# anibali/dsnt-pose2d

Measured on AMD Instinct MI355X. Metric: images/sec (train step, 256x256, 16 joints), higher is better.
Workload: dtype f32; 1 GPU; hg2 + DSNT + JS reg, 256x256 -> 64x64x16, batch 32 per GPU, RMSprop lr 2.5e-4, train step fwd+loss+bwd+optim; global_batch=32, parallelism=dp1, launches_fwd=212

## Files before the change

dsnt-pose2d_amd/csrc/elementwise.hip:

```cpp
#include "common.h"
#include <string.h>
#include "bn_pro.h"
#include "conv_split.h"
#include "ew_bodies.h"
#include "stage.h"

static inline int tile_cgs(long tiles, int C4) { return tiles < 256 && C4 > 16 && C4 % 16 == 0 ? 16 : (C4 < 256 ? C4 : 256); }
static inline unsigned tile_grid_y(long tiles, int C4) { const int c = tile_cgs(tiles, C4); return c == 16 && C4 > 16 ? C4 / 16 : 1; }

template <int MODE>
__global__ __launch_bounds__(256) void tile_reduce_kernel(
    const float* __restrict__ a, const float* __restrict__ x, const float* __restrict__ scale,
    const float* __restrict__ shift, const float* __restrict__ mean,
    const float* __restrict__ invstd, int relu, float* __restrict__ partial, long M, int C, int cgs,
    const float* __restrict__ ymask = nullptr, float* __restrict__ dz_out = nullptr) {
    __shared__ float red[256 * 8];
    const int tid = threadIdx.x;
    const int C4 = C >> 2;
    const int rpar = 256 / cgs;
    const int cg_l = tid % cgs, rl = tid / cgs;
    const bool active = rl < rpar;
    const long row0 = (long)blockIdx.x * TILE_ROWS;
    const long row1 = row0 + TILE_ROWS < M ? row0 + TILE_ROWS : M;
    for (int cg0 = blockIdx.y * cgs; cg0 < C4; cg0 += cgs * gridDim.y) {
// ... 294 lines not shown
        DSNT_LAUNCH_OP(DSNT_ST_APPLY, bn_act_bwd_apply_kernel<false>, dim3(grid), dim3(256), 0, stream, ap);
    DSNT_CHECK_LAUNCH("dsnt_bn_act_bwd_apply");
}

extern "C" int dsnt_bn_act_bwd_apply_pro(const float* da, const float* x, const float* scale, const float* shift,
                                         const float* mean, const float* invstd, const float* partial, int ntiles,
                                         float* dgamma, float* dbeta, int accumulate_params, float* coef, int relu,
                                         float* dx, int accumulate, int64_t M, int C, float* amax, void* stream) {
    DSNT_REQUIRE(partial && ntiles > 0 && coef && C <= 256 && (long)ntiles * C <= 16384, DSNT_ERR_ARG,
                 "dsnt_bn_act_bwd_apply_pro: needs partial sums of at most 256 channels / 128 KB and a coef buffer");
    BnBwdProP q;
    q.partial = partial; q.tiles = ntiles; q.C = C; q.invM = 1.0 / (double)M;
    q.dgamma = dgamma; q.dbeta = dbeta; q.accumulate = accumulate_params; q.coef = coef;
    return bn_act_bwd_apply_impl(da, x, scale, shift, mean, invstd, coef, relu, dx, accumulate, M, C, amax, stream, &q);
}
extern "C" int dsnt_bn_act_bwd_apply_base(const float* da, const float* x, const float* scale, const float* shift,
                                          const float* mean, const float* invstd, const float* coef, int relu,
                                          const float* base, float* dx, int64_t M, int C, float* amax, void* stream) {
    DSNT_REQUIRE(base && base != dx, DSNT_ERR_ARG, "dsnt_bn_act_bwd_apply_base: `base` must be a second tensor");
    return bn_act_bwd_apply_impl(da, x, scale, shift, mean, invstd, coef, relu, dx, 1, M, C, amax, stream, nullptr, base);
}
extern "C" int dsnt_bn_act_bwd_apply_pro_base(const float* da, const float* x, const float* scale, const float* shift,
                                              const float* mean, const float* invstd, const float* partial, int ntiles,
                                              float* dgamma, float* dbeta, int accumulate_params, float* coef, int relu,
                                              const float* base, float* dx, int64_t M, int C, float* amax, void* stream) {
    DSNT_REQUIRE(base && base != dx, DSNT_ERR_ARG, "dsnt_bn_act_bwd_apply_pro_base: `base` must be a second tensor");
    DSNT_REQUIRE(partial && ntiles > 0 && coef && C <= 256 && (long)ntiles * C <= 16384, DSNT_ERR_ARG,
                 "dsnt_bn_act_bwd_apply_pro_base: needs partial sums of at most 256 channels / 128 KB and a coef buffer");
    BnBwdProP q;
    q.partial = partial; q.tiles = ntiles; q.C = C; q.invM = 1.0 / (double)M;
    q.dgamma = dgamma; q.dbeta = dbeta; q.accumulate = accumulate_params; q.coef = coef;
    return bn_act_bwd_apply_impl(da, x, scale, shift, mean, invstd, coef, relu, dx, 1, M, C, amax, stream, &q, base);
}
__global__ void maxpool2_fwd_kernel(const float4* __restrict__ x, float4* __restrict__ y,
                                    uchar4* __restrict__ idx, int N, int H, int W, int C4) {
    const int Ho = H >> 1, Wo = W >> 1;
    const long total = (long)N * Ho * Wo * C4;
    for (long i = (long)blockIdx.x * blockDim.x + threadIdx.x; i < total;
         i += (long)gridDim.x * blockDim.x) {
        const int cg = (int)(i % C4);
        long t = i / C4;
        const int ow = (int)(t % Wo); t /= Wo;
        const int oh = (int)(t % Ho);
        const int n = (int)(t / Ho);
        const float4* base = x + (((long)n * H + 2 * oh) * W + 2 * ow) * C4 + cg;
        const float4 v0 = base[0], v1 = base[C4], v2 = base[(long)W * C4], v3 = base[(long)W * C4 + C4];
        float4 m = v0;
        uchar4 k = make_uchar4(0, 0, 0, 0);
#define POOL_STEP(V, P)                                  \
        if (V.x > m.x || V.x != V.x) { m.x = V.x; k.x = P; } \
        if (V.y > m.y || V.y != V.y) { m.y = V.y; k.y = P; } \
        if (V.z > m.z || V.z != V.z) { m.z = V.z; k.z = P; } \
        if (V.w > m.w || V.w != V.w) { m.w = V.w; k.w = P; }
        POOL_STEP(v1, 1) POOL_STEP(v2, 2) POOL_STEP(v3, 3)
#undef POOL_STEP
        y[i] = m;
        idx[i] = k;
    }
}

extern "C" int dsnt_maxpool2_fwd(const float* x, float* y, uint8_t* idx, int N, int H, int W, int C,
                                 void* stream) {
    DSNT_REQUIRE(x && y && idx && N > 0 && H > 0 && W > 0 && C > 0, DSNT_ERR_ARG, "dsnt_maxpool2_fwd: bad argument");
    DSNT_REQUIRE(H % 2 == 0 && W % 2 == 0, DSNT_ERR_SHAPE, "dsnt_maxpool2_fwd: H and W must be even (got %dx%d)", H, W);
    DSNT_REQUIRE(C % 4 == 0 && dsnt_aligned16(x) && dsnt_aligned16(y) && (((uintptr_t)idx) & 3) == 0,
                 DSNT_ERR_ALIGN, "dsnt_maxpool2_fwd: alignment");
// ... 548 lines not shown
```

dsnt-pose2d_amd/csrc/ew_bodies.h:

```cpp
#pragma once
#include "common.h"
#include "bn_pro.h"

#define TILE_ROWS 128

struct TileOpP {
    const float* a; const float* b; float* y; unsigned char* idx; float* partial;
    int N, Ho, Wo, C, cgs;
    OutBoundsP tail;
    const float* bn_scale; const float* bn_shift; int bn_relu;
};
template <int OP>
__device__ __forceinline__ void tile_op_stats_body(const TileOpP& q, const int bx, const int by, const int gy, float* red) {
    const float* __restrict__ a = q.a; const float* __restrict__ b = q.b; float* __restrict__ y = q.y;
    unsigned char* __restrict__ idx = q.idx; float* partial = q.partial;
    const int N = q.N, Ho = q.Ho, Wo = q.Wo, C = q.C, cgs = q.cgs;
    const OutBoundsP tail = q.tail;
    const float* __restrict__ bn_scale = q.bn_scale; const float* __restrict__ bn_shift = q.bn_shift; const int bn_relu = q.bn_relu;
    const int tid = threadIdx.x;
    const int C4 = C >> 2;
    const int rpar = 256 / cgs;
    const int cg_l = tid % cgs, rl = tid / cgs;
    const bool active = rl < rpar;
    const long M = (long)N * Ho * Wo;
// ... 93 lines not shown
                for (int e = 0; e < 8; ++e) acc[e] += red[(j * cgs + tid) * 8 + e];
            float* p0 = partial + ((size_t)bx * 2 + 0) * C + (size_t)(cg0 + tid) * 4;
            float* p1 = partial + ((size_t)bx * 2 + 1) * C + (size_t)(cg0 + tid) * 4;
            *reinterpret_cast<float4*>(p0) = make_float4(acc[0], acc[1], acc[2], acc[3]);
            *reinterpret_cast<float4*>(p1) = make_float4(acc[4], acc[5], acc[6], acc[7]);
        }
    }
    if (tail.amax) amax_commit(am, tail.amax, 0, bx);
    if (tail.amax_bn) amax_commit(am2, tail.amax_bn, 1, bx);
}

template <int OP>
__global__ __launch_bounds__(256) void tile_op_stats_kernel(TileOpP q) {
    __shared__ __attribute__((aligned(16))) float red[256 * 8];
    tile_op_stats_body<OP>(q, blockIdx.x, blockIdx.y, gridDim.y, red);
}

struct BnApplyVec { float4 sc, sh, mu, is, c0, c1; };
__device__ __forceinline__ float4 bn_apply_one(const float4 g, const float4 xv, const BnApplyVec& v, int relu) {
    float4 dz = g;
    if (relu) {
        if (fmaf(xv.x, v.sc.x, v.sh.x) <= 0.f) dz.x = 0.f;
        if (fmaf(xv.y, v.sc.y, v.sh.y) <= 0.f) dz.y = 0.f;
        if (fmaf(xv.z, v.sc.z, v.sh.z) <= 0.f) dz.z = 0.f;
        if (fmaf(xv.w, v.sc.w, v.sh.w) <= 0.f) dz.w = 0.f;
    }
    float4 o;
    o.x = v.sc.x * (dz.x - v.c0.x - (xv.x - v.mu.x) * v.is.x * v.c1.x);
    o.y = v.sc.y * (dz.y - v.c0.y - (xv.y - v.mu.y) * v.is.y * v.c1.y);
    o.z = v.sc.z * (dz.z - v.c0.z - (xv.z - v.mu.z) * v.is.z * v.c1.z);
    o.w = v.sc.w * (dz.w - v.c0.w - (xv.w - v.mu.w) * v.is.w * v.c1.w);
    return o;
}
struct BnApplyP {
    const float4* da; const float4* x; const float4* scale; const float4* shift; const float4* mean; const float4* invstd;
    const float4* coef; int relu; float4* dx; const float4* base; long n4; int C4; unsigned* amax; BnBwdProP pro;
};
template <bool FIXED>
__device__ __forceinline__ void bn_act_bwd_apply_body(const BnApplyP& q, const int vb, const int vgrid, double* pro_sh, const bool finalise) {
    const float4* __restrict__ da = q.da; const float4* __restrict__ x = q.x; const float4* __restrict__ scale = q.scale;
    const float4* __restrict__ shift = q.shift; const float4* __restrict__ mean = q.mean; const float4* __restrict__ invstd = q.invstd;
    const float4* coef = q.coef; const int relu = q.relu; float4* dx = q.dx; const float4* base = q.base;
    const long n4 = q.n4; const int C4 = q.C4; unsigned* __restrict__ amax = q.amax; const BnBwdProP pro = q.pro;
    const bool accumulate = base != nullptr;
    if (pro.partial && finalise) {
        bn_pro_backward<256>(pro, pro_sh, vb == 0);
        __syncthreads();
    }
    float am = 0.f;
    const long stride = (long)vgrid * 256;
    long i = threadIdx.x < 256 ? (long)vb * 256 + threadIdx.x : n4;
    auto vec = [&](int cg) {
        BnApplyVec v;
        v.sc = scale[cg]; v.sh = shift[cg]; v.mu = mean[cg]; v.is = invstd[cg]; v.c0 = coef[cg]; v.c1 = coef[C4 + cg];
        return v;
    };
    auto amx = [&](const float4 o) { am = fmaxf(fmaxf(fmaxf(fabsf(o.x), fabsf(o.y)), fmaxf(fabsf(o.z), fabsf(o.w))), am); };
    if (FIXED) {
        const BnApplyVec v = vec((int)((i < n4 ? i : 0) % C4));
        for (; i + stride < n4; i += 2 * stride) {
            const float4 g0 = da[i], x0 = x[i], g1 = da[i + stride], x1 = x[i + stride];
            float4 p0 = make_float4(0.f, 0.f, 0.f, 0.f), p1 = p0;
            if (accumulate) { p0 = base[i]; p1 = base[i + stride]; }
            float4 o0 = bn_apply_one(g0, x0, v, relu), o1 = bn_apply_one(g1, x1, v, relu);
            if (accumulate) {
                o0.x += p0.x; o0.y += p0.y; o0.z += p0.z; o0.w += p0.w;
                o1.x += p1.x; o1.y += p1.y; o1.z += p1.z; o1.w += p1.w;
            }
            dx[i] = o0; dx[i + stride] = o1;
            amx(o0); amx(o1);
        }
        if (i < n4) {
            float4 o = bn_apply_one(da[i], x[i], v, relu);
            if (accumulate) { const float4 p = base[i]; o.x += p.x; o.y += p.y; o.z += p.z; o.w += p.w; }
            dx[i] = o;
            amx(o);
        }
    } else {
        for (; i < n4; i += stride) {
            float4 o = bn_apply_one(da[i], x[i], vec((int)(i % C4)), relu);
            if (accumulate) { const float4 p = base[i]; o.x += p.x; o.y += p.y; o.z += p.z; o.w += p.w; }
            dx[i] = o;
            amx(o);
        }
    }
    if (amax) amax_commit(am, amax, 0, vb);
}

template <bool FIXED>
__global__ void bn_act_bwd_apply_kernel(BnApplyP q) {
    __shared__ double pro_sh[512];
    bn_act_bwd_apply_body<FIXED>(q, blockIdx.x, gridDim.x, pro_sh, true);
}

struct PoolBwdP { const float4* dy; const uchar4* idx; float4* dx; int accumulate; const float4* extra; int N, H, W, C4; unsigned* amax; };
__device__ __forceinline__ void maxpool2_bwd_body(const PoolBwdP& q, const int vb, const int vgrid) {
    const float4* __restrict__ dy = q.dy; const uchar4* __restrict__ idx = q.idx; float4* dx = q.dx; const int accumulate = q.accumulate;
    const float4* __restrict__ extra = q.extra; const int H = q.H, W = q.W, C4 = q.C4, N = q.N; unsigned* amax = q.amax;
    const int Ho = H >> 1, Wo = W >> 1;
    const long total = (long)N * Ho * Wo * C4;
    float am = 0.f;
    for (long i = threadIdx.x < 256 ? (long)vb * 256 + threadIdx.x : total; i < total; i += (long)vgrid * 256) {
        const int cg = (int)(i % C4);
        long t = i / C4;
        const int ow = (int)(t % Wo); t /= Wo;
        const int oh = (int)(t % Ho);
        const int n = (int)(t / Ho);
        const float4 g = dy[i];
        const uchar4 k = idx[i];
        float4* base = dx + (((long)n * H + 2 * oh) * W + 2 * ow) * C4 + cg;
#pragma unroll
        for (int p = 0; p < 4; ++p) {
            float4* q = base + (p >> 1) * (long)W * C4 + (p & 1) * C4;
            float4 o = make_float4(k.x == p ? g.x : 0.f, k.y == p ? g.y : 0.f, k.z == p ? g.z : 0.f,
                                   k.w == p ? g.w : 0.f);
            if (accumulate) { const float4 c = *q; o.x += c.x; o.y += c.y; o.z += c.z; o.w += c.w; }
            if (extra) { const float4 e = extra[q - dx]; o.x += e.x; o.y += e.y; o.z += e.z; o.w += e.w; }
            *q = o;
            am = fmaxf(fmaxf(fmaxf(fabsf(o.x), fabsf(o.y)), fmaxf(fabsf(o.z), fabsf(o.w))), am);
        }
    }
    if (amax) amax_commit(am, amax, 0, vb);
}

struct UpBwdP { const float4* dout; float4* dlow; int accumulate; int N, H, W, C4; unsigned* amax; };
// ... 124 lines not shown
```

dsnt-pose2d_amd/dsnt/_lib.py:

```python
import ctypes as C
import os

import torch

_HERE = os.path.dirname(os.path.abspath(__file__))
LIB_PATH = os.environ.get('DSNT_HIP_LIB') or os.path.join(os.path.dirname(_HERE), 'csrc', 'libdsnt_hip.so')

P = C.c_void_p
I = C.c_int
L = C.c_int64
F = C.c_float
D = C.c_double


class ConvGeom(C.Structure):
    _fields_ = [(n, C.c_int) for n in
                ('N', 'H', 'W', 'Cin', 'Ho', 'Wo', 'Cout', 'R', 'S', 'stride', 'pad', 'dil')]


GP = C.POINTER(ConvGeom)


class BnBwdEpilogue(C.Structure):
    _fields_ = [('x', C.c_void_p), ('scale', C.c_void_p), ('shift', C.c_void_p), ('mean', C.c_void_p),
# ... 63 lines not shown
    'dsnt_conv_fwd_bf16x6_ex': [P, P, L, P, P, P, P, I, P, P, P, GP, BP, TP, P],
    'dsnt_conv_pack_dgrad': [P, P, I, I, I, I, P],
    'dsnt_conv_pack_dgrad_all': [P, I, P, P, P, L, P],
    'dsnt_conv_fwd_bf16x6': [P, P, L, P, P, P, P, I, P, P, P, GP, P],
    'dsnt_split_bf16x3': [P, P, L, P],
    'dsnt_conv_fwd_f16x3_ex': [P, P, L, P, P, P, P, P, P, I, P, P, P, GP, BP, TP, P],
    'dsnt_conv_fwd_f16x3_stream': [P, P, L, P, P, P, P, P, P, I, P, P, P, GP, BP, TP, P],
    'dsnt_amax': [P, L, P, P],
    'dsnt_split_f16x2': [P, P, L, L, P, P],
    'dsnt_f16_prep_weights': [P, I, I, P],
    'dsnt_f16_prep_bn_bounds': [P, I, P],
    'dsnt_conv_wgrad': [P, P, P, I, P, P, P, P, I, GP, P],
    'dsnt_conv_wgrad_bf16x6': [P, P, P, I, P, P, P, P, I, GP, P],
    'dsnt_conv_wgrad_f16x3': [P, P, P, I, P, P, P, P, I, P, P, GP, P],
    'dsnt_conv1x1_fwd_f16x3': [P, P, L, P, P, P, P, P, P, I, P, P, GP, TP, P],
    'dsnt_conv1x1_bwd_f16x3': [BP, P, AP, P, L, P, P, P, P, P, P, P, I, GP, P],
    'dsnt_conv_dgrad_f16x3_stream_apply': [P, AP, P, P, L, P, P, P, P, I, GP, BP, TP, P],
    'dsnt_wgrad_reduce_all': [P, I, I, P],
    'dsnt_conv_wgrad_group': [P, I, I, P],
    'dsnt_bn_stats': [P, P, L, I, P],
    'dsnt_bn_finalize': [P, I, L, I, P, P, P, P, F, F, I, P, P, P, P, P],
    'dsnt_bn_act_fwd': [P, P, P, I, P, L, I, P],
    'dsnt_bn_act_bwd_reduce': [P, P, P, P, P, P, I, P, L, I, P],
    'dsnt_bn_bwd_finalize': [P, I, L, I, P, P, I, P, P],
    'dsnt_bn_bwd_finalize_bound': [P, I, L, I, P, P, I, P, P, P, P, P],
    'dsnt_bn_eval_prep': [P, I, P],
    'dsnt_bn_act_bwd_apply': [P, P, P, P, P, P, P, I, P, I, L, I, P],
    'dsnt_bn_act_bwd_apply_amax': [P, P, P, P, P, P, P, I, P, I, L, I, P, P],
    'dsnt_bn_act_bwd_apply_pro': [P, P, P, P, P, P, P, I, P, P, I, P, I, P, I, L, I, P, P],
    'dsnt_stem4_fwd_f16x3': [P, P, L, P, P, P, P, P, GP, TP, P],
    'dsnt_bn_add_act_bwd_reduce': [P, P, P, P, P, I, P, P, L, I, P],
    'dsnt_bn_act_bwd_apply_base': [P, P, P, P, P, P, P, I, P, P, L, I, P, P],
    'dsnt_bn_act_bwd_apply_pro_base': [P, P, P, P, P, P, P, I, P, P, I, P, I, P, P, L, I, P, P],
    'dsnt_conv_fwd_pro': [P, P, P, P, PP, I, P, P, P, GP, TP, P],
    'dsnt_fill_zero': [P, L, P],
    'dsnt_axpy_amax': [P, P, F, I, L, P, P],
    'dsnt_maxpool2_bwd_amax': [P, P, P, I, I, I, I, I, P, P],
    'dsnt_maxpool2_bwd_add': [P, P, P, I, P, I, I, I, I, P, P],
    'dsnt_upsample2_bwd_amax': [P, P, I, I, I, I, I, P, P],
    'dsnt_maxpool2_fwd': [P, P, P, I, I, I, I, P],
    'dsnt_maxpool2_bwd': [P, P, P, I, I, I, I, I, P],
    'dsnt_maxpool2_fwd_stats': [P, P, P, P, I, I, I, I, TP, P],
    'dsnt_upsample2_add_fwd_stats': [P, P, P, P, I, I, I, I, TP, P],
    'dsnt_bn_act_fwd_stats': [P, P, P, I, P, P, L, I, TP, P],
    'dsnt_s2d_input': [P, P, I, I, I, I, TP, P],
    'dsnt_s2d_weights': [P, P, I, I, P],
    'dsnt_s2d_weights_prep': [P, P, P, P, P, I, P],
    'dsnt_maxpool3s2_fwd': [P, P, P, I, I, I, I, P],
    'dsnt_maxpool3s2_bwd': [P, P, P, I, I, I, I, I, P],
    'dsnt_bn_add_act_fwd': [P, P, P, P, I, P, L, I, P],
    'dsnt_relu_bwd': [P, P, P, L, P],
    'dsnt_zero_insert': [P, P, I, I, I, I, I, I, I, P],
    'dsnt_conv_dgrad_strided': [P, P, P, P, P, GP, BP, TP, P],
    'dsnt_upsample2_add_fwd': [P, P, P, I, I, I, I, P],
    'dsnt_upsample2_bwd': [P, P, I, I, I, I, I, P],
    'dsnt_axpy': [P, P, F, I, L, P],
    'dsnt_nchw_to_nhwc': [P, P, I, I, I, I, P],
    'dsnt_nhwc_to_nchw': [P, P, I, I, I, I, P],
    'dsnt_rmsprop_step': [P, P, P, L, F, F, F, F, F, P],
    'dsnt_sgd_step': [P, P, P, L, F, F, F, F, I, P],
    'dsnt_rmsprop_step_guarded': [P, P, P, L, F, F, F, F, F, P, P],
    'dsnt_sgd_step_guarded': [P, P, P, L, F, F, F, F, I, P, P],
    'dsnt_nonfinite_flag': [P, L, P, I, P],
    'dsnt_pckh': [P, P, P, P, P, P, F, P, P, I, I, P],
    'dsnt_pckh_hist': [P, P, P, P, P, P, P, I, P, P, I, I, P],
    'dsnt_augment_fwd': [P, I, I, I, P, P, P, P, I, C.c_uint64, C.c_uint64, P, P, P, P],
# ... 115 lines not shown
```

dsnt-pose2d_amd/dsnt/engine.py:

```python
import ctypes as C
import os

import torch

from . import _lib
from ._lib import ConvGeom, BnBwdEpilogue, BnTail, BnPrologue, BnBwdApply

BN_EPS = 1e-5
BN_MOMENTUM = 0.1


class Act:
    __slots__ = ('buf', 'N', 'H', 'W', 'C', '_grad', 'stats', 'name', 'grad_amax', 'amax_tail', 'fold_ok',
                 'pending_apply', 'uses', 'gives_away', 'is_branch', 'grad_shared', 'pending_add', 'base', 'base_amax')

    def __init__(self, buf, name=''):
        self.buf = buf
        self.N, self.H, self.W, self.C = buf.shape
        self._grad = None
        self.base, self.base_amax = None, None
        self.stats = None
        self.amax_tail = None
        self.grad_amax = None
        self.fold_ok = False
        self.pending_apply = None
        self.uses = 0
        self.gives_away = False
        self.is_branch = False
        self.grad_shared = False
        self.pending_add = None
        self.name = name

    @property
    def M(self):
        return self.N * self.H * self.W

    @property
    def grad(self):
        if self._grad is None and self.base is not None:
            self._grad, self.grad_amax, self.grad_shared = self.base, self.base_amax, True
        return self._grad

    @grad.setter
    def grad(self, g):
        self._grad = g


class ConvParams:
    __slots__ = ('w', 'b', 'gw', 'gb', 'Cout', 'R', 'S', 'Cin', 'stride', 'pad', 'dil', 'wq', 'wq_stride', 'wq16', 'wb',
                 'post_reduce')

    def __init__(self, w, b, gw, gb, stride=1, pad=0, dil=1):
        self.w, self.b, self.gw, self.gb = w, b, gw, gb
        self.wq, self.wq_stride = None, 0
        self.wq16, self.wb = None, None
        self.post_reduce = None
        self.Cout, self.R, self.S, self.Cin = w.shape
        self.stride, self.pad, self.dil = stride, pad, dil


class BnParams:
    __slots__ = ('gamma', 'beta', 'ggamma', 'gbeta', 'rmean', 'rvar', 'C', 'uses', 'momentum', 'eps')

# ... 13 lines not shown
    def __init__(self, device, training, record=None):
        self.device = device
        self.training = training
        self.record = training if record is None else bool(record)
        self.fwd = []
        self.bwd = []
        self._bwd_emitters = []
        self._scratch = {}
        self._keep = []
        self.lib = _lib.load()
        self.nbytes = 0
        self.bytes_fwd, self.bytes_bwd, self.bytes_by_name, self._ws_ptrs = 0, 0, {}, set()
        self.use_bf16x6 = os.environ.get('DSNT_MFMA', 'bf16x6') != 'f32'
        self.bf16x6_min_rows = int(os.environ.get('DSNT_BF16X6_MIN_ROWS', '4096'))
        self.lane = 0
        self.use_lanes = os.environ.get('DSNT_LANES', '1') != '0'
        self.fuse_join = True
        self.side_stream = None
        self.wgrad_stream = None
        self.side_lanes = (1, 3)
        self.n_lanes = 3 + len(self.side_lanes) - 1
        self.chain_lanes = (0,) + self.side_lanes
        self.more_streams = ()
        self.wgrad_lane = 2 if (self.use_lanes and os.environ.get('DSNT_WGRAD_LANE', '1') != '0') else None
        self.wgrad_lane_rows = int(os.environ.get('DSNT_X_WGRAD_LANE_ROWS', '16000'))
        self.wgrad_lane_res = False
        self.wgrad_lane_from = self.chain_lanes
        self.conv3s = 'conv3s' not in os.environ.get('DSNT_OFF', '').replace('+', ',').split(',')
        self.bwd1 = 'bwd1' not in os.environ.get('DSNT_OFF', '').replace('+', ',').split(',')
        self.fwd1 = 'fwd1' not in os.environ.get('DSNT_OFF', '').replace('+', ',').split(',')
        self.fold3 = 'fold3' not in os.environ.get('DSNT_OFF', '').replace('+', ',').split(',')
        self.fold3_rows = int(os.environ.get('DSNT_X_FOLD3_ROWS', '16384'))
        self.stem4 = 'stem4' not in os.environ.get('DSNT_OFF', '').replace('+', ',').split(',')
        self.stage = os.environ.get('DSNT_STAGE', '0') == '1'
        self.stage_min_run = int(os.environ.get('DSNT_X_STAGE_MIN_RUN', '3'))
        self.stage_max_vgrid = int(os.environ.get('DSNT_X_STAGE_MAX_VGRID', '512'))
        self.stage_grid = int(os.environ.get('DSNT_X_STAGE_GRID', '64'))
        self.stage_census = []
        self._f16_w_stream = {}
        self.conv_share = True
        self.wgrad_share = True
        self._x = dict(kv.split('=') for kv in os.environ.get('DSNT_X', '').split(',') if '=' in kv)
        self.wgrad_narrow = self._x.get('wgrad_narrow', '1')
        self.share_grads = self._x.get('share_grads', '1') != '0'
        self.defer_res = self._x.get('defer_res', '1') != '0'
        self.flush_points = self._x.get('flush_points', '1') != '0'
        self.prep_split = self._x.get('prep_split', '1') != '0'
        self.cur_bucket = 0
        self._wgrad_lane_reads = set()
        self._writer_base = None
        self._ident = None
        self.release_rows = int(os.environ.get('DSNT_X_RELEASE_ROWS', '4096'))
        self._release_total, self._release_left = 0, 0
        self._held = []
        self.acts = []
        self.dgrad_slots = []
        self.dgrad_total = 0
        self.dgrad_f32 = None
        self.dgrad_planes = None
        self.param_arena = None
        self.defer_reduce = os.environ.get('DSNT_DEFER_REDUCE', '1') != '0'
        self._pending_reduce = []
        self.group_rows = int(os.environ.get('DSNT_X_GROUP_ROWS', '8192')) if self.defer_reduce else 0
        self._pending_group = []
        self.fuse_op_stats = True
        self.fuse_finalize = os.environ.get('DSNT_FUSE_FINALIZE', '1') != '0'
        self.fuse_finalize_max = int(os.environ.get('DSNT_X_FUSE_FINALIZE_MAX', '2048'))
        self.use_f16x3 = self.use_bf16x6 and os.environ.get('DSNT_SPLIT', 'f16x3') == 'f16x3'
        if self.record and not self.training:
            self.use_f16x3 = False
        self._f16_w_rows, self._f16_w_seen = [], set()
        self._f16_bn_rows = []
        self._eval_bn_rows = []
        self._amax_buf, self._amax_used = None, 0
        self.raw_f16 = True
        self._planar_src, self._prep_exempt, self._post_reduce = {}, set(), []
        self.stem_s2d_on = True
        self._famax_buf, self._famax_used, self._famax_of, self._famax_bn_of = None, 0, {}, {}
        self.amax_all = True
        self._f16_dw_rows = []
        self._dgrad_pack = None
        self.prep_on_side_lane = self.use_lanes
        self.dgrad_planes16, self.dgrad_bounds = None, None
        self.f16_uses = []
        self._pending_group_uses = []
        self.c_replay = True
        self._clists = {}

    def empty(self, *shape, dtype=torch.float32):
        t = torch.empty(*shape, device=self.device, dtype=dtype)
        self.nbytes += t.numel() * t.element_size()
        self._keep.append(t)
        return t

    def scratch(self, key, numel):
        if False:
            return self.empty(max(numel, 1))
        key = (key, self.lane)
        t = self._scratch.get(key)
        if t is None or t.numel() < numel:
            if t is not None:
                self._keep.append(t)
            t = torch.empty(max(numel, 1), device=self.device, dtype=torch.float32)
            self.nbytes += t.numel() * 4
            self._scratch[key] = t
        return t

    def scratch_bf16(self, key, numel):
        key = (key, self.lane)
        t = self._scratch.get(key)
        if t is None or t.numel() < numel:
            if t is not None:
                self._keep.append(t)
            t = torch.empty(max(numel, 8), device=self.device, dtype=torch.bfloat16)
            self.nbytes += t.numel() * 2
            self._scratch[key] = t
        return t

    def f16_weights(self, p, wq16=None, wsrc=None, wb=None, stream=False):
        wq16 = p.wq16 if wq16 is None else wq16
        key = wq16.data_ptr()
        if key not in self._f16_w_seen:
            self._f16_w_seen.add(key)
            wsrc = p.w if wsrc is None else wsrc
            wb = p.wb if wb is None else wb
            n = wsrc.numel()
            assert n % 4 == 0
            self._f16_w_rows.append([wsrc.data_ptr(), wq16.data_ptr(), wb.data_ptr(), n, p.wq_stride] +
                                    ([p.Cout, p.Cin] if stream else [0, 0]))
            self._f16_w_stream[key] = stream
# ... 483 lines not shown
                self.f('dsnt_bn_finalize', part, tiles, x.M, bn.C, bn.gamma, bn.beta, bn.rmean, bn.rvar,
                       bn.momentum, bn.eps, 1, n.mean, n.invstd, n.scale, n.shift)
        else:
            import struct
            bits = struct.unpack('<I', struct.pack('<f', float(bn.eps)))[0]
            self._eval_bn_rows.append([bn.gamma.data_ptr(), bn.beta.data_ptr(), bn.rmean.data_ptr(), bn.rvar.data_ptr(),
                                       n.mean.data_ptr(), n.invstd.data_ptr(), n.scale.data_ptr(), n.shift.data_ptr(),
                                       bn.C, bits])
        return n

    def check_lane(self, n):
        if n.pending is not None:
            n.lane = self.lane
        elif n.lane != self.lane:
            raise RuntimeError('dsnt: BatchNorm vectors finalised on lane %d are read on lane %d without a synchronisation '
                               '(trace norm() and its consumers on one lane, or sync the lanes)' % (n.lane, self.lane))

    def materialize(self, n):
        self.check_lane(n)
        if n.pending is not None:
            part, tiles = n.pending
            n.pending = None
            bn = n.bn
            self.f('dsnt_bn_finalize', part, tiles, n.x.M, bn.C, bn.gamma, bn.beta, bn.rmean, bn.rvar,
                   bn.momentum, bn.eps, 1, n.mean, n.invstd, n.scale, n.shift)

    def fold_ok(self, n):
        x = n.x
        return bool(self.bwd1 and x.fold_ok and x.grad is None and x.pending_apply is None)

    def materialize_apply(self, x):
        ap, x.pending_apply = x.pending_apply, None
        n = ap['n']
        buf, acc = self.grad_target(x, amax='apply')
        if x.grad_amax is not None:
            self.b('dsnt_bn_act_bwd_apply_amax', ap['dz'], x.buf, n.scale, n.shift, n.mean, n.invstd, ap['coef'], 0,
                   buf, acc, x.M, n.bn.C, x.grad_amax)
        else:
            self.b('dsnt_bn_act_bwd_apply', ap['dz'], x.buf, n.scale, n.shift, n.mean, n.invstd, ap['coef'], 0,
                   buf, acc, x.M, n.bn.C)

    def _norm_backward(self, n, da, reduced=None, finalised=False, dz_amax=None):
        x, bn = n.x, n.bn
        coef = self.scratch('bncoef', 2 * bn.C)
        relu = 1 if n.relu else 0
        if reduced is not None:
            part, tiles = reduced
            relu = 0
        else:
            tiles = (x.M + 127) // 128
            part = self.scratch('bnpart', tiles * 2 * bn.C).view(-1)
            self.b('dsnt_bn_act_bwd_reduce', da, x.buf, n.scale, n.shift, n.mean, n.invstd, relu, part,
                   x.M, bn.C)
        if dz_amax is not None:
            assert reduced is not None and not finalised and x.grad is None
            acc_p = 1 if bn.uses > 0 else 0
            bn.uses += 1
            coef = self.empty(2 * bn.C)
            bound = self.amax_slot()
            self.b('dsnt_bn_bwd_finalize_bound', part, tiles, x.M, bn.C, bn.ggamma, bn.gbeta, acc_p, coef, n.scale,
                   dz_amax, bound)
            x.pending_apply = dict(dz=da, n=n, coef=coef, bound=bound, dz_amax=dz_amax)
            return
        frozen = not self.training
        fused = (not finalised) and self.fuse_finalize and bn.C <= 256 and tiles * bn.C <= self.fuse_finalize_max and not frozen
        assert not (frozen and finalised)
        if not finalised:
            acc_p = 1 if bn.uses > 0 else 0
            bn.uses += 1
            if not fused:
                self.b('dsnt_bn_bwd_finalize', part, tiles, x.M, bn.C, bn.ggamma, bn.gbeta, acc_p | (2 if frozen else 0), coef)
        buf, acc = self.grad_target(x, amax='apply', base_ok=True)
        base = self.take_base()
        if fused:
            coef = self.empty(2 * bn.C)
            if base is not None:
                self.b('dsnt_bn_act_bwd_apply_pro_base', da, x.buf, n.scale, n.shift, n.mean, n.invstd, part, tiles,
                       bn.ggamma, bn.gbeta, acc_p, coef, relu, base, buf, x.M, bn.C, x.grad_amax)
            else:
                self.b('dsnt_bn_act_bwd_apply_pro', da, x.buf, n.scale, n.shift, n.mean, n.invstd, part, tiles,
                       bn.ggamma, bn.gbeta, acc_p, coef, relu, buf, acc, x.M, bn.C, x.grad_amax)
        elif base is not None:
            self.b('dsnt_bn_act_bwd_apply_base', da, x.buf, n.scale, n.shift, n.mean, n.invstd, coef, relu,
                   base, buf, x.M, bn.C, x.grad_amax)
        elif x.grad_amax is not None:
            self.b('dsnt_bn_act_bwd_apply_amax', da, x.buf, n.scale, n.shift, n.mean, n.invstd, coef, relu,
                   buf, acc, x.M, bn.C, x.grad_amax)
        else:
            self.b('dsnt_bn_act_bwd_apply', da, x.buf, n.scale, n.shift, n.mean, n.invstd, coef, relu,
                   buf, acc, x.M, bn.C)

    def conv(self, src, p, res1=None, res2=None, want_stats=False, need_input_grad=True, name=''):
        normed = isinstance(src, Normed)
        x = src.x if normed else src
        g = self.geom(x, p)
        y = self.act(x.N, g.Ho, g.Wo, p.Cout, name)
        x.uses += 1
        for r in (res1, res2):
            if r is not None:
                r.uses += 1
                y.gives_away = True
        sc = src.scale if normed else None
        sh = src.shift if normed else None
        relu = 1 if (normed and src.relu) else 0
        if normed:
            self.check_lane(src)
        part, tail = None, None
        use6 = self._use6(g) and p.wq is not None
# ... 344 lines not shown
        if self.training and self.fuse_op_stats:
            tiles = (y.M + 127) // 128
            part = self.empty(tiles, 2, x.C)
            y.amax_tail = BnTail() if big else None
            self.f('dsnt_bn_act_fwd_stats', x.buf, n.scale, n.shift, 1 if n.relu else 0, y.buf, part, x.M, x.C, y.amax_tail)
            y.stats = (part, tiles)
        elif not self.training and big:
            y.amax_tail = BnTail()
            self.f('dsnt_bn_act_fwd_stats', x.buf, n.scale, n.shift, 1 if n.relu else 0, y.buf, None, x.M, x.C, y.amax_tail)
        else:
            self.f('dsnt_bn_act_fwd', x.buf, n.scale, n.shift, 1 if n.relu else 0, y.buf, x.M, x.C)
        if self.record:
            def backward():
                self._norm_backward(n, y.grad)
            self.on_backward(backward)
        return y

    def maxpool2(self, x, name=''):
        y = self.act(x.N, x.H // 2, x.W // 2, x.C, name)
        x.uses += 1
        idx = self.empty(x.N, x.H // 2, x.W // 2, x.C, dtype=torch.uint8)
        if self.training and self.fuse_op_stats:
            tiles = (y.M + 127) // 128
            part = self.empty(tiles, 2, x.C)
            y.amax_tail = BnTail() if (self.use_f16x3 and y.M >= self.bf16x6_min_rows) else None
            self.f('dsnt_maxpool2_fwd_stats', x.buf, y.buf, idx, part, x.N, x.H, x.W, x.C, y.amax_tail)
            y.stats = (part, tiles)
        elif not self.training and self.use_f16x3 and y.M >= self.bf16x6_min_rows:
            y.amax_tail = BnTail()
            self.f('dsnt_maxpool2_fwd_stats', x.buf, y.buf, idx, None, x.N, x.H, x.W, x.C, y.amax_tail)
        else:
            self.f('dsnt_maxpool2_fwd', x.buf, y.buf, idx, x.N, x.H, x.W, x.C)
        if self.record:
            def backward():
                add, x.pending_add = x.pending_add, None
                buf, acc = self.grad_target(x, amax=True, take_add=True)
                if add is not None:
                    assert acc == 1
                    self.b('dsnt_maxpool2_bwd_add', y.grad, idx, buf, acc, add[0], x.N, x.H, x.W, x.C, x.grad_amax)
                elif x.grad_amax is not None:
                    self.b('dsnt_maxpool2_bwd_amax', y.grad, idx, buf, acc, x.N, x.H, x.W, x.C, x.grad_amax)
                else:
                    self.b('dsnt_maxpool2_bwd', y.grad, idx, buf, acc, x.N, x.H, x.W, x.C)
            self.on_backward(backward)
        return y

    def maxpool3s2(self, x, name=''):
        Ho, Wo = (x.H - 1) // 2 + 1, (x.W - 1) // 2 + 1
        y = self.act(x.N, Ho, Wo, x.C, name)
        x.uses += 1
        idx = self.empty(x.N, Ho, Wo, x.C, dtype=torch.uint8)
        self.f('dsnt_maxpool3s2_fwd', x.buf, y.buf, idx, x.N, x.H, x.W, x.C)
        if self.record:
            def backward():
                buf, acc = self.grad_target(x)
                self.b('dsnt_maxpool3s2_bwd', y.grad, idx, buf, acc, x.N, x.H, x.W, x.C)
            self.on_backward(backward)
        return y

    def bn_add_act(self, x, bn, skip, relu=True, name=''):
        n = self.norm(x, bn, relu=False)
        y = self.act(x.N, x.H, x.W, x.C, name)
        x.uses += 1
        skip.uses += 1
        if os.environ.get('DSNT_DEBUG_NO_RELU'):
            relu = False
        self.materialize(n)
        self.f('dsnt_bn_add_act_fwd', x.buf, n.scale, n.shift, skip.buf, 1 if relu else 0, y.buf, x.M, x.C)
        if self.record:
            def backward():
# ... 5 lines not shown
                    part = self.scratch('bnpart', tiles * 2 * bn.C).view(-1)
                    self.b('dsnt_bn_add_act_bwd_reduce', y.grad, y.buf, x.buf, n.mean, n.invstd, 1, dz, part, x.M, bn.C)
                    self._norm_backward(n, dz, reduced=(part, tiles))
                else:
                    dz = y.grad
                    self._norm_backward(n, dz)
                if share and skip._grad is None and skip.base is None:
                    skip.base, skip.base_amax = dz, None
                else:
                    self.grad_identity(skip, dz, donate=False)
            self.on_backward(backward)
        return y

    def upsample2_add(self, up, low, name=''):
        out = self.act(up.N, up.H, up.W, up.C, name)
        up.uses += 1
        low.uses += 1
        out.gives_away = True
        if self.training and self.fuse_op_stats:
            tiles = (out.M + 127) // 128
            part = self.empty(tiles, 2, up.C)
            out.amax_tail = BnTail() if (self.use_f16x3 and out.M >= self.bf16x6_min_rows) else None
            self.f('dsnt_upsample2_add_fwd_stats', up.buf, low.buf, out.buf, part, up.N, up.H, up.W, up.C, out.amax_tail)
            out.stats = (part, tiles)
        elif not self.training and self.use_f16x3 and out.M >= self.bf16x6_min_rows:
            out.amax_tail = BnTail()
            self.f('dsnt_upsample2_add_fwd_stats', up.buf, low.buf, out.buf, None, up.N, up.H, up.W, up.C, out.amax_tail)
        else:
            self.f('dsnt_upsample2_add_fwd', up.buf, low.buf, out.buf, up.N, up.H, up.W, up.C)
        if self.record:
            point = self.wgrad_lane is not None and low.M <= self.release_rows
            self._release_total += point

            def backward():
                if point:
                    self._release_left -= 1
                    self.release_wgrads()
                buf, acc = self.grad_target(low, amax=True)
                if low.grad_amax is not None:
                    self.b('dsnt_upsample2_bwd_amax', out.grad, buf, acc, up.N, up.H, up.W, up.C, low.grad_amax)
                else:
                    self.b('dsnt_upsample2_bwd', out.grad, buf, acc, up.N, up.H, up.W, up.C)
                self.grad_identity(up, out.grad, donate=True, g_amax=out.grad_amax)
            self.on_backward(backward)
        return out

    def to_planar(self, x, C_logical, name='', out=None, gin=None):
        out = self.empty(x.N, C_logical, x.H, x.W) if out is None else out
        x.uses += 1
        if gin is None:
            gin = self.empty(x.N, C_logical, x.H, x.W) if self.record else None
        self.f('dsnt_nhwc_to_nchw', x.buf, out, x.N, C_logical, x.H * x.W, x.C)
        if self.record:
            def backward():
                assert x.grad is None, 'planar output must be the first gradient writer'
                buf, _ = self.grad_target(x)
                self.b('dsnt_nchw_to_nhwc', gin, buf, x.N, C_logical, x.H * x.W, x.C)
            self.on_backward(backward)
        return out, gin

    def from_planar(self, src_nchw, Cpad, name=''):
        N, Cc, H, W = src_nchw.shape
        a = self.act(N, H, W, Cpad, name)
        e = self.f('dsnt_nchw_to_nhwc', src_nchw, a.buf, N, Cc, H * W, Cpad)
        self._planar_src[id(a)] = (src_nchw, e)
        return a

    def stem_s2d(self, x, p, name='stem'):
        got = self._planar_src.get(id(x))
        if (got is None or not self.use_f16x3 or not self.stem_s2d_on or p.R != 7 or p.S != 7 or p.stride != 2 or p.pad != 3
                or p.dil != 1 or x.C != 4 or x.H % 2 or x.W % 2 or x.N * (x.H // 2) * (x.W // 2) < self.bf16x6_min_rows):
            return None
# ... 18 lines not shown
```

include/dsnt_hip.h:

```cpp
#ifndef DSNT_HIP_H
#define DSNT_HIP_H

#include <stdint.h>

#ifdef __cplusplus
extern "C" {
#endif

typedef enum {
    DSNT_OK = 0,
    DSNT_ERR_SHAPE = 1,
    DSNT_ERR_ALIGN = 2,
    DSNT_ERR_ARG = 3,
    DSNT_ERR_HIP = 4
} dsnt_status;

typedef struct {
    float* amax;
    float* amax_bn; const float* amax_scale; const float* amax_shift; int amax_relu, reserved;
} dsnt_out_bounds;

typedef struct dsnt_bn_prologue {
    const float* partial; int tiles, C;
    int64_t M;
// ... 216 lines not shown
                    float* y, int64_t M, int C, void* stream);

int dsnt_bn_eval_prep(const int64_t* table, int rows, void* stream);
#define DSNT_BN_FROZEN 2
int dsnt_bn_act_bwd_reduce(const float* da, const float* x, const float* scale,
                           const float* shift, const float* mean, const float* invstd,
                           int relu, float* partial, int64_t M, int C, void* stream);
int dsnt_bn_add_act_bwd_reduce(const float* da, const float* y, const float* x, const float* mean, const float* invstd,
                               int relu, float* dz, float* partial, int64_t M, int C, void* stream);
int dsnt_bn_bwd_finalize(const float* partial, int ntiles, int64_t M, int C,
                         float* dgamma, float* dbeta, int accumulate, float* coef,
                         void* stream);
int dsnt_bn_bwd_finalize_bound(const float* partial, int ntiles, int64_t M, int C, float* dgamma, float* dbeta,
                               int accumulate, float* coef, const float* scale, const float* dz_amax, float* bound_out,
                               void* stream);
int dsnt_bn_act_bwd_apply(const float* da, const float* x, const float* scale,
                          const float* shift, const float* mean, const float* invstd,
                          const float* coef, int relu, float* dx, int accumulate,
                          int64_t M, int C, void* stream);
int dsnt_bn_act_bwd_apply_amax(const float* da, const float* x, const float* scale, const float* shift,
                               const float* mean, const float* invstd, const float* coef, int relu, float* dx,
                               int accumulate, int64_t M, int C, float* amax, void* stream);
int dsnt_bn_act_bwd_apply_pro(const float* da, const float* x, const float* scale, const float* shift,
                              const float* mean, const float* invstd, const float* partial, int ntiles,
                              float* dgamma, float* dbeta, int accumulate_params, float* coef, int relu,
                              float* dx, int accumulate, int64_t M, int C, float* amax, void* stream);
int dsnt_bn_act_bwd_apply_base(const float* da, const float* x, const float* scale, const float* shift,
                               const float* mean, const float* invstd, const float* coef, int relu,
                               const float* base, float* dx, int64_t M, int C, float* amax, void* stream);
int dsnt_bn_act_bwd_apply_pro_base(const float* da, const float* x, const float* scale, const float* shift,
                                   const float* mean, const float* invstd, const float* partial, int ntiles,
                                   float* dgamma, float* dbeta, int accumulate_params, float* coef, int relu,
                                   const float* base, float* dx, int64_t M, int C, float* amax, void* stream);
int dsnt_fill_zero(float* p, int64_t n, void* stream);
int dsnt_axpy_amax(const float* x, float* y, float a, int accumulate, int64_t n, float* amax, void* stream);
int dsnt_maxpool2_bwd_amax(const float* dy, const uint8_t* idx, float* dx, int accumulate, int N, int H, int W, int C,
                           float* amax, void* stream);
int dsnt_maxpool2_bwd_add(const float* dy, const uint8_t* idx, float* dx, int accumulate, const float* extra,
                          int N, int H, int W, int C, float* amax, void* stream);
int dsnt_upsample2_bwd_amax(const float* dout, float* dlow, int accumulate, int N, int H, int W, int C, float* amax,
                            void* stream);

int dsnt_maxpool2_fwd(const float* x, float* y, uint8_t* idx, int N, int H, int W, int C,
                      void* stream);
int dsnt_maxpool2_bwd(const float* dy, const uint8_t* idx, float* dx, int accumulate,
                      int N, int H, int W, int C, void* stream);

int dsnt_maxpool3s2_fwd(const float* x, float* y, uint8_t* idx, int N, int H, int W, int C, void* stream);
int dsnt_maxpool3s2_bwd(const float* dy, const uint8_t* idx, float* dx, int accumulate, int N, int H, int W,
                        int C, void* stream);
int dsnt_bn_add_act_fwd(const float* x, const float* scale, const float* shift, const float* res, int relu,
                        float* y, int64_t M, int C, void* stream);
int dsnt_relu_bwd(const float* dy, const float* y, float* dz, int64_t n, void* stream);
int dsnt_zero_insert(const float* dy, float* out, int N, int Ho, int Wo, int C, int Hs, int Ws, int stride,
                     void* stream);

int dsnt_conv_dgrad_strided(const float* dy, const float* wd, float* dx, const float* res1, float* stats_partial,
                            const dsnt_conv_geom* g, const dsnt_bn_bwd_epilogue* bnb, const dsnt_out_bounds* tail, void* stream);
int dsnt_conv_dgrad_strided_ok(const dsnt_conv_geom* g);
int dsnt_conv_dgrad_strided_tiles(const dsnt_conv_geom* g);

int dsnt_upsample2_add_fwd(const float* up, const float* low, float* out,
                           int N, int H, int W, int C, void* stream);
int dsnt_upsample2_bwd(const float* dout, float* dlow, int accumulate,
                       int N, int H, int W, int C, void* stream);

// ... 102 lines not shown
```

Measured before the change: 2881 images/sec.

## Fuse BN backward apply with upsample2/maxpool2 backward via deferred route

Adds kernels that apply the batch-norm+ReLU backward and, in the same pass, route the resulting gradient through the 2x upsample backward (summing 2x2 blocks into the low-res grad) or the 2x2 maxpool backward (scattering by argmax index). The engine defers the BN apply on the upsample/pool output until the corresponding backward runs, then emits a single fused launch. This is meant to remove one kernel launch and a full re-read of the high-resolution gradient per fused site. In exchange it adds deferred-state bookkeeping that must be flushed before scratch reuse, and the pool path is off by default. Each thread now handles four pixels, which reduces parallelism.

New measurement: 2892 images/sec (median of 6 runs). Within noise of the previous version (+0.4%).

```diff
diff --git a/dsnt-pose2d_amd/csrc/elementwise.hip b/dsnt-pose2d_amd/csrc/elementwise.hip
--- a/dsnt-pose2d_amd/csrc/elementwise.hip
+++ b/dsnt-pose2d_amd/csrc/elementwise.hip
@@ -350,6 +350,75 @@
     q.dgamma = dgamma; q.dbeta = dbeta; q.accumulate = accumulate_params; q.coef = coef;
     return bn_act_bwd_apply_impl(da, x, scale, shift, mean, invstd, coef, relu, dx, 1, M, C, amax, stream, &q, base);
 }
+
+template <int ROUTE>
+static int bn_apply_route_launch(const char* who, BnApplyP ap, const float* partial, int ntiles, float* dgamma, float* dbeta,
+                                 int accumulate_params, int64_t M, int C, void* stream) {
+    const BnRouteP& r = ap.route;
+    DSNT_REQUIRE(ap.da && ap.x && ap.scale && ap.shift && ap.mean && ap.invstd && ap.coef && r.dst && r.N > 0 && r.H > 0 && r.W > 0 &&
+                 C > 0, DSNT_ERR_ARG, "%s: bad argument", who);
+    DSNT_REQUIRE(r.H % 2 == 0 && r.W % 2 == 0, DSNT_ERR_SHAPE, "%s: H and W must be even (got %dx%d)", who, r.H, r.W);
+    DSNT_REQUIRE(C % 4 == 0 && dsnt_aligned16(ap.da) && dsnt_aligned16(ap.x) && dsnt_aligned16(ap.dx) && dsnt_aligned16(ap.coef) &&
+                 dsnt_aligned16(ap.base) && dsnt_aligned16(ap.scale) && dsnt_aligned16(ap.shift) && dsnt_aligned16(ap.mean) &&
+                 dsnt_aligned16(ap.invstd) && dsnt_aligned16(r.dst) && dsnt_aligned16(r.extra) && (((uintptr_t)r.idx) & 3) == 0,
+                 DSNT_ERR_ALIGN, "%s: alignment", who);
+    memset(&ap.pro, 0, sizeof(ap.pro));
+    if (partial) {
+        DSNT_REQUIRE(ntiles > 0 && C <= 256 && (long)ntiles * C <= 16384, DSNT_ERR_ARG,
+                     "%s: the prologue needs partial sums of at most 256 channels / 128 KB", who);
+        ap.pro.partial = partial; ap.pro.tiles = ntiles; ap.pro.C = C; ap.pro.invM = 1.0 / (double)M;
+        ap.pro.dgamma = dgamma; ap.pro.dbeta = dbeta; ap.pro.accumulate = accumulate_params; ap.pro.coef = (float*)ap.coef;
+    }
+    ap.C4 = C / 4;
+    ap.n4 = (long)M * ap.C4;
+    const long owned = (long)r.N * (r.H / 2) * (r.W / 2) * ap.C4;
+    int grid = flat_grid(owned, 256);
+    if (partial && grid > 128) grid = 128;
+    hipStream_t st = (hipStream_t)stream;
+    if (((long)grid * 256) % ap.C4 == 0)
+        DSNT_LAUNCH((bn_act_bwd_apply_route_kernel<true, ROUTE>), dim3(grid), dim3(256), 0, st, ap);
+    else
+        DSNT_LAUNCH((bn_act_bwd_apply_route_kernel<false, ROUTE>), dim3(grid), dim3(256), 0, st, ap);
+    DSNT_CHECK_LAUNCH(who);
+}
+
+extern "C" int dsnt_bn_act_bwd_apply_up2(const float* da, const float* x, const float* scale, const float* shift, const float* mean,
+                                         const float* invstd, const float* partial, int ntiles, float* dgamma, float* dbeta,
+                                         int accumulate_params, float* coef, int relu, const float* base, float* dx, int accumulate,
+                                         float* dlow, int accumulate_low, int N, int H, int W, int C, float* amax, float* amax_low,
+                                         void* stream) {
+    const char* who = "dsnt_bn_act_bwd_apply_up2";
+    DSNT_REQUIRE(dx && dlow && dlow != dx, DSNT_ERR_ARG, "%s: bad argument", who);
+    DSNT_REQUIRE(base != dx && !(base && accumulate), DSNT_ERR_ARG, "%s: `base` must be a second tensor (in place: accumulate)", who);
+    BnApplyP ap;
+    memset(&ap, 0, sizeof(ap));
+    ap.da = (const float4*)da; ap.x = (const float4*)x; ap.scale = (const float4*)scale; ap.shift = (const float4*)shift;
+    ap.mean = (const float4*)mean; ap.invstd = (const float4*)invstd; ap.coef = (const float4*)coef; ap.relu = relu;
+    ap.dx = (float4*)dx; ap.base = (const float4*)(accumulate ? dx : base); ap.amax = (unsigned*)amax;
+    ap.route.dst = (float4*)dlow; ap.route.accumulate = accumulate_low; ap.route.amax = (unsigned*)amax_low;
+    ap.route.N = N; ap.route.H = H; ap.route.W = W;
+    return bn_apply_route_launch<BN_ROUTE_SUM>(who, ap, partial, ntiles, dgamma, dbeta, accumulate_params, (int64_t)N * H * W, C, stream);
+}
+
+extern "C" int dsnt_bn_act_bwd_apply_pool2(const float* da, const float* x, const float* scale, const float* shift, const float* mean,
+                                           const float* invstd, const float* partial, int ntiles, float* dgamma, float* dbeta,
+                                           int accumulate_params, float* coef, int relu, const float* base, const uint8_t* idx,
+                                           float* dx, int accumulate, const float* extra, int N, int H, int W, int C, float* amax,
+                                           void* stream) {
+    const char* who = "dsnt_bn_act_bwd_apply_pool2";
+    DSNT_REQUIRE(dx && idx, DSNT_ERR_ARG, "%s: bad argument", who);
+    DSNT_REQUIRE(base != dx && da != dx && extra != dx, DSNT_ERR_ARG, "%s: `base`, `da` and `extra` must be tensors of their own", who);
+    BnApplyP ap;
+    memset(&ap, 0, sizeof(ap));
+    ap.da = (const float4*)da; ap.x = (const float4*)x; ap.scale = (const float4*)scale; ap.shift = (const float4*)shift;
+    ap.mean = (const float4*)mean; ap.invstd = (const float4*)invstd; ap.coef = (const float4*)coef; ap.relu = relu;
+    ap.base = (const float4*)base;
+    ap.route.dst = (float4*)dx; ap.route.idx = (const uchar4*)idx; ap.route.extra = (const float4*)extra;
+    ap.route.accumulate = accumulate; ap.route.amax = (unsigned*)amax;
+    ap.route.N = N; ap.route.H = H; ap.route.W = W;
+    return bn_apply_route_launch<BN_ROUTE_SCATTER>(who, ap, partial, ntiles, dgamma, dbeta, accumulate_params,
+                                                   (int64_t)N * (H / 2) * (W / 2), C, stream);
+}
 __global__ void maxpool2_fwd_kernel(const float4* __restrict__ x, float4* __restrict__ y,
                                     uchar4* __restrict__ idx, int N, int H, int W, int C4) {
     const int Ho = H >> 1, Wo = W >> 1;
diff --git a/dsnt-pose2d_amd/csrc/ew_bodies.h b/dsnt-pose2d_amd/csrc/ew_bodies.h
--- a/dsnt-pose2d_amd/csrc/ew_bodies.h
+++ b/dsnt-pose2d_amd/csrc/ew_bodies.h
@@ -149,9 +149,11 @@
     o.w = v.sc.w * (dz.w - v.c0.w - (xv.w - v.mu.w) * v.is.w * v.c1.w);
     return o;
 }
+enum { BN_ROUTE_SUM = 1, BN_ROUTE_SCATTER = 2 };
+struct BnRouteP { float4* dst; const uchar4* idx; const float4* extra; unsigned* amax; int accumulate, N, H, W; };
 struct BnApplyP {
     const float4* da; const float4* x; const float4* scale; const float4* shift; const float4* mean; const float4* invstd;
-    const float4* coef; int relu; float4* dx; const float4* base; long n4; int C4; unsigned* amax; BnBwdProP pro;
+    const float4* coef; int relu; float4* dx; const float4* base; long n4; int C4; unsigned* amax; BnBwdProP pro; BnRouteP route;
 };
 template <bool FIXED>
 __device__ __forceinline__ void bn_act_bwd_apply_body(const BnApplyP& q, const int vb, const int vgrid, double* pro_sh, const bool finalise) {
@@ -208,6 +210,85 @@
 __global__ void bn_act_bwd_apply_kernel(BnApplyP q) {
     __shared__ double pro_sh[512];
     bn_act_bwd_apply_body<FIXED>(q, blockIdx.x, gridDim.x, pro_sh, true);
+}
+
+__device__ __forceinline__ float4 add4_rounded(const float4 a, const float4 b) {
+#pragma clang fp contract(off)
+    return make_float4(a.x + b.x, a.y + b.y, a.z + b.z, a.w + b.w);
+}
+template <bool FIXED, int ROUTE>
+__device__ __forceinline__ void bn_act_bwd_apply_route_body(const BnApplyP& q, const int vb, const int vgrid, double* pro_sh) {
+    const float4* __restrict__ da = q.da; const float4* __restrict__ x = q.x; const float4* __restrict__ scale = q.scale;
+    const float4* __restrict__ shift = q.shift; const float4* __restrict__ mean = q.mean; const float4* __restrict__ invstd = q.invstd;
+    const float4* coef = q.coef; const int relu = q.relu; float4* dx = q.dx; const float4* base = q.base;
+    const int C4 = q.C4; unsigned* __restrict__ amax = q.amax; const BnBwdProP pro = q.pro; const BnRouteP r = q.route;
+    const bool accumulate = base != nullptr;
+    const int H = r.H, W = r.W, Hl = H >> 1, Wl = W >> 1;
+    const long total = (long)r.N * Hl * Wl * C4;
+    if (pro.partial) {
+        bn_pro_backward<256>(pro, pro_sh, vb == 0);
+        __syncthreads();
+    }
+    float am = 0.f, am2 = 0.f;
+    const long stride = (long)vgrid * 256;
+    long i = (long)vb * 256 + threadIdx.x;
+    auto vec = [&](int cg) {
+        BnApplyVec v;
+        v.sc = scale[cg]; v.sh = shift[cg]; v.mu = mean[cg]; v.is = invstd[cg]; v.c0 = coef[cg]; v.c1 = coef[C4 + cg];
+        return v;
+    };
+    auto amx = [](const float4 o, float& m) { m = fmaxf(fmaxf(fmaxf(fabsf(o.x), fabsf(o.y)), fmaxf(fabsf(o.z), fabsf(o.w))), m); };
+    BnApplyVec v = vec((int)((i < total ? i : 0) % C4));
+    for (; i < total; i += stride) {
+        const int cg = (int)(i % C4);
+        long t = i / C4;
+        const int w = (int)(t % Wl); t /= Wl;
+        const int h = (int)(t % Hl);
+        const int n = (int)(t / Hl);
+        if (!FIXED) v = vec(cg);
+        const long f0 = (((long)n * H + 2 * h) * W + 2 * w) * C4 + cg;
+        if (ROUTE == BN_ROUTE_SUM) {
+            float4 g[4], xv[4], p[4], o[4];
+#pragma unroll
+            for (int k = 0; k < 4; ++k) {
+                const long f = f0 + (k >> 1) * (long)W * C4 + (k & 1) * C4;
+                g[k] = da[f]; xv[k] = x[f];
+                p[k] = accumulate ? base[f] : make_float4(0.f, 0.f, 0.f, 0.f);
+            }
+#pragma unroll
+            for (int k = 0; k < 4; ++k) {
+                o[k] = bn_apply_one(g[k], xv[k], v, relu);
+                if (accumulate) { o[k].x += p[k].x; o[k].y += p[k].y; o[k].z += p[k].z; o[k].w += p[k].w; }
+                dx[f0 + (k >> 1) * (long)W * C4 + (k & 1) * C4] = o[k];
+                amx(o[k], am);
+            }
+            float4 s = add4_rounded(add4_rounded(o[0], o[1]), add4_rounded(o[2], o[3]));
+            if (r.accumulate) s = add4_rounded(s, r.dst[i]);
+            r.dst[i] = s;
+            amx(s, am2);
+        } else {
+            float4 o = bn_apply_one(da[i], x[i], v, relu);
+            if (accumulate) { const float4 p = base[i]; o.x += p.x; o.y += p.y; o.z += p.z; o.w += p.w; }
+            const uchar4 k = r.idx[i];
+#pragma unroll
+            for (int p = 0; p < 4; ++p) {
+                const long f = f0 + (p >> 1) * (long)W * C4 + (p & 1) * C4;
+                float4 s = make_float4(k.x == p ? o.x : 0.f, k.y == p ? o.y : 0.f, k.z == p ? o.z : 0.f, k.w == p ? o.w : 0.f);
+                if (r.accumulate) s = add4_rounded(s, r.dst[f]);
+                if (r.extra) s = add4_rounded(s, r.extra[f]);
+                r.dst[f] = s;
+                amx(s, am2);
+            }
+        }
+    }
+    if (amax) amax_commit(am, amax, 0, vb);
+    if (r.amax) amax_commit(am2, r.amax, 1, vb);
+}
+
+template <bool FIXED, int ROUTE>
+__global__ __launch_bounds__(256) void bn_act_bwd_apply_route_kernel(BnApplyP q) {
+    __shared__ double pro_sh[512];
+    bn_act_bwd_apply_route_body<FIXED, ROUTE>(q, blockIdx.x, gridDim.x, pro_sh);
 }
 
 struct PoolBwdP { const float4* dy; const uchar4* idx; float4* dx; int accumulate; const float4* extra; int N, H, W, C4; unsigned* amax; };
diff --git a/dsnt-pose2d_amd/dsnt/_lib.py b/dsnt-pose2d_amd/dsnt/_lib.py
--- a/dsnt-pose2d_amd/dsnt/_lib.py
+++ b/dsnt-pose2d_amd/dsnt/_lib.py
@@ -119,6 +119,8 @@
     'dsnt_bn_add_act_bwd_reduce': [P, P, P, P, P, I, P, P, L, I, P],
     'dsnt_bn_act_bwd_apply_base': [P, P, P, P, P, P, P, I, P, P, L, I, P, P],
     'dsnt_bn_act_bwd_apply_pro_base': [P, P, P, P, P, P, P, I, P, P, I, P, I, P, P, L, I, P, P],
+    'dsnt_bn_act_bwd_apply_up2': [P, P, P, P, P, P, P, I, P, P, I, P, I, P, P, I, P, I, I, I, I, I, P, P, P],
+    'dsnt_bn_act_bwd_apply_pool2': [P, P, P, P, P, P, P, I, P, P, I, P, I, P, P, P, I, P, I, I, I, I, P, P],
     'dsnt_conv_fwd_pro': [P, P, P, P, PP, I, P, P, P, GP, TP, P],
     'dsnt_fill_zero': [P, L, P],
     'dsnt_axpy_amax': [P, P, F, I, L, P, P],
diff --git a/dsnt-pose2d_amd/dsnt/engine.py b/dsnt-pose2d_amd/dsnt/engine.py
--- a/dsnt-pose2d_amd/dsnt/engine.py
+++ b/dsnt-pose2d_amd/dsnt/engine.py
@@ -12,7 +12,7 @@
 
 class Act:
     __slots__ = ('buf', 'N', 'H', 'W', 'C', '_grad', 'stats', 'name', 'grad_amax', 'amax_tail', 'fold_ok',
-                 'pending_apply', 'uses', 'gives_away', 'is_branch', 'grad_shared', 'pending_add', 'base', 'base_amax')
+                 'pending_apply', 'uses', 'gives_away', 'is_branch', 'grad_shared', 'pending_add', 'base', 'base_amax', 'route')
 
     def __init__(self, buf, name=''):
         self.buf = buf
@@ -29,6 +29,7 @@
         self.is_branch = False
         self.grad_shared = False
         self.pending_add = None
+        self.route = None
         self.name = name
 
     @property
@@ -108,6 +109,9 @@
         self.fold3 = 'fold3' not in os.environ.get('DSNT_OFF', '').replace('+', ',').split(',')
         self.fold3_rows = int(os.environ.get('DSNT_X_FOLD3_ROWS', '16384'))
         self.stem4 = 'stem4' not in os.environ.get('DSNT_OFF', '').replace('+', ',').split(',')
+        _parts = os.environ.get('DSNT_X_ROUTE', 'up').split(',')
+        self.route_up, self.route_pool = 'up' in _parts, 'pool' in _parts
+        self._route_open = None
         self.stage = os.environ.get('DSNT_STAGE', '0') == '1'
         self.stage_min_run = int(os.environ.get('DSNT_X_STAGE_MIN_RUN', '3'))
         self.stage_max_vgrid = int(os.environ.get('DSNT_X_STAGE_MAX_VGRID', '512'))
@@ -172,6 +176,8 @@
     def scratch(self, key, numel):
         if False:
             return self.empty(max(numel, 1))
+        if self._route_open is not None and self._route_open.pending_apply['lane'] == self.lane:
+            self.materialize_apply(self._route_open)
         key = (key, self.lane)
         t = self._scratch.get(key)
         if t is None or t.numel() < numel:
@@ -721,6 +727,10 @@
     def materialize_apply(self, x):
         ap, x.pending_apply = x.pending_apply, None
         n = ap['n']
+        if ap.get('route'):
+            self._route_open = None
+            self._emit_apply(n, ap['dz'], ap['coef'], ap['relu'], ap['pro'])
+            return
         buf, acc = self.grad_target(x, amax='apply')
         if x.grad_amax is not None:
             self.b('dsnt_bn_act_bwd_apply_amax', ap['dz'], x.buf, n.scale, n.shift, n.mean, n.invstd, ap['coef'], 0,
@@ -759,10 +769,36 @@
             bn.uses += 1
             if not fused:
                 self.b('dsnt_bn_bwd_finalize', part, tiles, x.M, bn.C, bn.ggamma, bn.gbeta, acc_p | (2 if frozen else 0), coef)
+        pro = (part, tiles, acc_p) if fused else None
+        if fused:
+            coef = self.empty(2 * bn.C)
+        kind, lane = x.route if x.route is not None else (None, None)
+        if ((self.route_up if kind == 'up2' else self.route_pool if kind == 'pool2' else False) and not frozen and lane == self.lane and
+                x.pending_apply is None and x.pending_add is None and self._route_open is None):
+            x.pending_apply = dict(route=kind, lane=lane, n=n, dz=da, coef=coef, relu=relu, pro=pro)
+            self._route_open = x
+            return
+        self._emit_apply(n, da, coef, relu, pro)
+
+    def _emit_apply(self, n, da, coef, relu, pro, route=None):
+        x, bn = n.x, n.bn
+        fused = pro is not None
+        part, tiles, acc_p = pro if fused else (None, 0, 0)
+        if route is not None and route[0] == 'pool2':
+            base, x.base, x.base_amax = (x.base if x._grad is None else x._grad), None, None
+            _, idx, dst, acc, extra, slot = route
+            self.b('dsnt_bn_act_bwd_apply_pool2', da, x.buf, n.scale, n.shift, n.mean, n.invstd, part, tiles,
+                   bn.ggamma if fused else None, bn.gbeta if fused else None, acc_p, coef, relu, base, idx, dst, acc, extra,
+                   x.N, 2 * x.H, 2 * x.W, bn.C, slot)
+            return
         buf, acc = self.grad_target(x, amax='apply', base_ok=True)
         base = self.take_base()
-        if fused:
-            coef = self.empty(2 * bn.C)
+        if route is not None:
+            _, dlow, acc_low, slot = route
+            self.b('dsnt_bn_act_bwd_apply_up2', da, x.buf, n.scale, n.shift, n.mean, n.invstd, part, tiles,
+                   bn.ggamma if fused else None, bn.gbeta if fused else None, acc_p, coef, relu, base, buf,
+                   acc if base is None else 0, dlow, acc_low, x.N, x.H, x.W, bn.C, x.grad_amax, slot)
+        elif fused:
             if base is not None:
                 self.b('dsnt_bn_act_bwd_apply_pro_base', da, x.buf, n.scale, n.shift, n.mean, n.invstd, part, tiles,
                        bn.ggamma, bn.gbeta, acc_p, coef, relu, base, buf, x.M, bn.C, x.grad_amax)
@@ -1173,10 +1209,21 @@
         else:
             self.f('dsnt_maxpool2_fwd', x.buf, y.buf, idx, x.N, x.H, x.W, x.C)
         if self.record:
+            y.route = ('pool2', self.lane)
+
             def backward():
+                ap = y.pending_apply
+                if ap is not None and not (ap.get('route') == 'pool2' and ap['lane'] == self.lane):
+                    self.materialize_apply(y)
+                    ap = None
                 add, x.pending_add = x.pending_add, None
                 buf, acc = self.grad_target(x, amax=True, take_add=True)
-                if add is not None:
+                if ap is not None:
+                    assert add is None or acc == 1
+                    y.pending_apply, self._route_open = None, None
+                    self._emit_apply(ap['n'], ap['dz'], ap['coef'], ap['relu'], ap['pro'],
+                                     route=('pool2', idx, buf, acc, add[0] if add is not None else None, x.grad_amax))
+                elif add is not None:
                     assert acc == 1
                     self.b('dsnt_maxpool2_bwd_add', y.grad, idx, buf, acc, add[0], x.N, x.H, x.W, x.C, x.grad_amax)
                 elif x.grad_amax is not None:
@@ -1248,12 +1295,21 @@
             point = self.wgrad_lane is not None and low.M <= self.release_rows
             self._release_total += point
 
+            out.route = ('up2', self.lane)
+
             def backward():
                 if point:
                     self._release_left -= 1
                     self.release_wgrads()
+                ap = out.pending_apply
+                if ap is not None and not (ap.get('route') == 'up2' and ap['lane'] == self.lane):
+                    self.materialize_apply(out)
+                    ap = None
                 buf, acc = self.grad_target(low, amax=True)
-                if low.grad_amax is not None:
+                if ap is not None:
+                    out.pending_apply, self._route_open = None, None
+                    self._emit_apply(ap['n'], ap['dz'], ap['coef'], ap['relu'], ap['pro'], route=('up2', buf, acc, low.grad_amax))
+                elif low.grad_amax is not None:
                     self.b('dsnt_upsample2_bwd_amax', out.grad, buf, acc, up.N, up.H, up.W, up.C, low.grad_amax)
                 else:
                     self.b('dsnt_upsample2_bwd', out.grad, buf, acc, up.N, up.H, up.W, up.C)
diff --git a/include/dsnt_hip.h b/include/dsnt_hip.h
--- a/include/dsnt_hip.h
+++ b/include/dsnt_hip.h
@@ -272,6 +272,16 @@
                                    const float* mean, const float* invstd, const float* partial, int ntiles,
                                    float* dgamma, float* dbeta, int accumulate_params, float* coef, int relu,
                                    const float* base, float* dx, int64_t M, int C, float* amax, void* stream);
+int dsnt_bn_act_bwd_apply_up2(const float* da, const float* x, const float* scale, const float* shift, const float* mean,
+                              const float* invstd, const float* partial, int ntiles, float* dgamma, float* dbeta,
+                              int accumulate_params, float* coef, int relu, const float* base, float* dx, int accumulate,
+                              float* dlow, int accumulate_low, int N, int H, int W, int C, float* amax, float* amax_low,
+                              void* stream);
+int dsnt_bn_act_bwd_apply_pool2(const float* da, const float* x, const float* scale, const float* shift, const float* mean,
+                                const float* invstd, const float* partial, int ntiles, float* dgamma, float* dbeta,
+                                int accumulate_params, float* coef, int relu, const float* base, const uint8_t* idx,
+                                float* dx, int accumulate, const float* extra, int N, int H, int W, int C, float* amax,
+                                void* stream);
 int dsnt_fill_zero(float* p, int64_t n, void* stream);
 int dsnt_axpy_amax(const float* x, float* y, float a, int accumulate, int64_t n, float* amax, void* stream);
 int dsnt_maxpool2_bwd_amax(const float* dy, const uint8_t* idx, float* dx, int accumulate, int N, int H, int W, int C,
```
